# Kitware/pyLiDAR-SLAM

Hardware: NVIDIA H100
Metric: icp_odometry_frames_per_sec (higher is better)
Workload: dtype f32

## Files before the change

pylidar_slam_b200/csrc/context.cu:

```cuda
#include <utility>

#include "internal.cuh"
#include "kdmap_device.cuh"

namespace pls {

long long g_kernel_launches = 0;

void DBuf::reserve(size_t bytes, cudaStream_t s, bool keep) {
    if (bytes <= cap) return;
    size_t want = bytes + bytes / 2 + 256;
    void* np = nullptr;
    PLS_CUDA(cudaStreamSynchronize(s));
    PLS_CUDA(cudaMalloc(&np, want));
    if (p) {
        if (keep) PLS_CUDA(cudaMemcpy(np, p, cap, cudaMemcpyDeviceToDevice));
        PLS_CUDA(cudaFree(p));
    }
    p = np;
    cap = want;
}

void DBuf::reserve_exact(size_t bytes, cudaStream_t s, bool keep) {
    if (bytes <= cap) return;
// ... 148 lines not shown
    cudaEventRecord(e0, ctx->stream);
}

ProfileScope::~ProfileScope() {
    if (e1) cudaEventRecord(e1, ctx->stream);
}

void profile_collect(pls_context* ctx, int which) {
    ProfileSlot& s = ctx->prof[which];
    for (size_t i = 0; i + 1 < s.used; i += 2) {
        float ms = 0.f;
        if (cudaEventElapsedTime(&ms, s.pool[i], s.pool[i + 1]) == cudaSuccess) s.ms += ms;
    }
    s.used = 0;
}

}

using namespace pls;

extern "C" {

const char* pls_version(void) { return "plslam_b200 0.1 (sm_90a)"; }

int pls_host_fingerprint(const void* host_ptr, int64_t num_bytes, uint64_t* out) {
    if (!host_ptr || !out || num_bytes < 0) return PLS_E_INVALID;
    const int64_t words = num_bytes / 8;
    uint64_t h = 0x9E3779B97F4A7C15ull ^ (uint64_t)num_bytes;
    const uint64_t* w = reinterpret_cast<const uint64_t*>(host_ptr);
    const int64_t step = words > 256 ? words / 256 : 1;
    for (int64_t i = 0; i < words; i += step) {
        uint64_t v;
        memcpy(&v, w + i, 8);
        h = (h ^ v) * 0x100000001B3ull;
        h ^= h >> 29;
    }
    if (words > 0) {
        uint64_t v;
        memcpy(&v, w + words - 1, 8);
        h = (h ^ v) * 0x100000001B3ull;
    }
    *out = h;
    return PLS_OK;
}

int pls_launch_count(int64_t* out) {
    if (!out) return PLS_E_INVALID;
    *out = (int64_t)pls::g_kernel_launches;
    return PLS_OK;
}

int pls_config_default(pls_config* c) {
    if (!c) return PLS_E_INVALID;
    memset(c, 0, sizeof(*c));
    c->height = 64;
    c->width = 2048;
    c->up_fov_deg = 3.0f;
    c->down_fov_deg = -24.0f;
    c->local_map_type = PLS_MAP_KDTREE;
    c->local_map_size = 20;
    c->num_neighbors_normals = 10;
    c->normals_kernel_size = 5;
    c->scheme = PLS_SCHEME_DEFAULT;
    c->sigma = 0.5f;
    c->gn_max_iters = 1;
    c->gn_norm_stop = 1e-3f;
    c->max_num_alignments = 100;
    c->threshold_delta_pose = 1e-4f;
    c->threshold_trans = 0.1f;
    c->threshold_rot = 0.3f;
    c->device = 0;
    c->stream = nullptr;
    return PLS_OK;
}

int pls_create(const pls_config* cfg, pls_context** out) {
    if (!cfg || !out) return PLS_E_INVALID;
    *out = nullptr;
    int ndev = 0;
    if (cudaGetDeviceCount(&ndev) != cudaSuccess || ndev <= 0) {
        cudaGetLastError();
        return PLS_E_CUDA;
    }
    if (cfg->device < 0 || cfg->device >= ndev) return PLS_E_INVALID;
    if (cfg->height <= 0 || cfg->width <= 0 || cfg->local_map_size <= 0) return PLS_E_INVALID;
    if (cfg->max_num_alignments < 1 || cfg->max_num_alignments > kMaxAlign) return PLS_E_INVALID;
    if (cfg->num_neighbors_normals < 3 || cfg->num_neighbors_normals + 1 > KD_KMAX_WIDE) return PLS_E_INVALID;
    if (cfg->normals_kernel_size < 1 || cfg->normals_kernel_size > 9 || (cfg->normals_kernel_size % 2) == 0)
        return PLS_E_INVALID;
    pls_context* ctx = new pls_context();
    ctx->cfg = *cfg;
    try {
        PLS_CUDA(cudaSetDevice(cfg->device));
        if (cfg->stream) {
            ctx->stream = (cudaStream_t)cfg->stream;
        } else {
            static const bool prio = !(getenv("PLS_STREAM_PRIORITY") && atoi(getenv("PLS_STREAM_PRIORITY")) == 0);
            int least = 0, greatest = 0;
            PLS_CUDA(cudaDeviceGetStreamPriorityRange(&least, &greatest));
            PLS_CUDA(cudaStreamCreateWithPriority(&ctx->stream, cudaStreamNonBlocking, prio ? greatest : 0));
            ctx->own_stream = true;
        }
        ctx->stream_main = ctx->stream;
        {
            static const bool prio = !(getenv("PLS_STREAM_PRIORITY") && atoi(getenv("PLS_STREAM_PRIORITY")) == 0);
            int least = 0, greatest = 0;
            PLS_CUDA(cudaDeviceGetStreamPriorityRange(&least, &greatest));
            PLS_CUDA(cudaStreamCreateWithPriority(&ctx->stream_map, cudaStreamNonBlocking, prio ? least : 0));
        }
        PLS_CUDA(cudaEventCreateWithFlags(&ctx->ev_map_done, cudaEventDisableTiming));
        ctx->pinned.reserve(kScalarOffset + 256);
        ctx->scalars.reserve(sizeof(FrameResult) + 4096, ctx->stream);
        PLS_CUDA(cudaMemsetAsync(ctx->scalars.p, 0, ctx->scalars.cap, ctx->stream));
        odometry_reset(ctx);
    } catch (const pls::Error& e) {
        fprintf(stderr, "pls_create: %s\n", e.msg.c_str());
        delete ctx;
        return e.code;
    }
    *out = ctx;
    return PLS_OK;
}

int pls_destroy(pls_context* ctx) {
    if (!ctx) return PLS_E_INVALID;
    cudaSetDevice(ctx->cfg.device);
    ctx->upd_pending = false;
    cudaStreamSynchronize(ctx->stream_map);
    cudaStreamSynchronize(ctx->stream_main);
    comm_free(ctx);
    if (ctx->p2p_pending_xchg) cudaFree(ctx->p2p_pending_xchg);
    for (auto& b : ctx->stage_in) b.release();
    for (auto& b : ctx->stage_out) b.release();
    for (auto& b : ctx->tmp) b.release();
    for (auto& b : ctx->next_buf) b.release();
    ctx->pinned.release();
    ctx->scalars.release();
    ctx->sort.keys_alt.release(); ctx->sort.vals_alt.release(); ctx->sort.hist.release();
    ctx->sort.status.release(); ctx->sort.plan.release();
    ctx->sort_map.keys_alt.release(); ctx->sort_map.vals_alt.release(); ctx->sort_map.hist.release();
    ctx->sort_map.status.release(); ctx->sort_map.plan.release();
    ctx->scan.status.release();
    ctx->sel[0].status.release(); ctx->sel[1].status.release(); ctx->input_zbuf.release();
    for (auto& b : ctx->kd.store) b.release();
    ctx->kd.morton.release(); ctx->kd.order.release(); ctx->kd.sorted.release(); ctx->kd.sorted_prev.release(); ctx->kd.normals.release();
    ctx->kd.bbox.release(); ctx->kd.grid_hdr.release(); ctx->kd.cells.release(); ctx->kd.stats.release();
    ctx->kd_worklist.release(); ctx->kd_nn_state.release();
    ctx->pm.vmaps.release(); ctx->pm.nmaps.release(); ctx->pm.poses.release();
    ctx->pm.model_v.release(); ctx->pm.model_n.release(); ctx->pm.zbuf.release();
    for (auto& b : ctx->frame_vmap_buf) b.release();
    for (auto& b : ctx->frame_pts_buf) b.release();
    ctx->queries.release(); ctx->nn_prev.release();
    ctx->partials.release(); ctx->batch_buf.release(); ctx->hyp_buf.release(); ctx->degen_buf.release(); ctx->gs_keys.release(); ctx->gs_vals.release(); ctx->gs_out_xyz.release();
    ctx->gs_out_idx.release();
    for (auto& s : ctx->prof)
        for (auto e : s.pool) cudaEventDestroy(e);
    if (ctx->ev_map_done) cudaEventDestroy(ctx->ev_map_done);
    if (ctx->ev_inputs) cudaEventDestroy(ctx->ev_inputs);
    if (ctx->ev_batch) cudaEventDestroy(ctx->ev_batch);
    if (ctx->ev_icp_done) cudaEventDestroy(ctx->ev_icp_done);
    ctx->gs_host_xyz.release(); ctx->gs_host_idx.release();
    if (ctx->stream_map) cudaStreamDestroy(ctx->stream_map);
    if (ctx->own_stream) cudaStreamDestroy(ctx->stream_main);
    delete ctx;
    return PLS_OK;
}

const char* pls_last_error(pls_context* ctx) { return ctx ? ctx->err.c_str() : "null context"; }

int pls_synchronize(pls_context* ctx) {
    PLS_API_BEGIN(ctx)
    sync_all(ctx);
    PLS_API_END(ctx)
}

int pls_wait_stream(pls_context* ctx, void* other_stream) {
    PLS_API_BEGIN(ctx)
    cudaStream_t other = (cudaStream_t)other_stream;
    if (other != ctx->stream_main) {
        if (!ctx->ev_inputs) PLS_CUDA(cudaEventCreateWithFlags(&ctx->ev_inputs, cudaEventDisableTiming));
        PLS_CUDA(cudaEventRecord(ctx->ev_inputs, other));
        PLS_CUDA(cudaStreamWaitEvent(ctx->stream_main, ctx->ev_inputs, 0));
    }
    PLS_API_END(ctx)
}

int pls_profile_enable(pls_context* ctx, int which, int enable) {
    PLS_API_BEGIN(ctx)
    PLS_REQUIRE(which >= 0 && which < kProfileSlots, "pls_profile_enable: bad slot");
    ctx->prof[which].enabled = enable != 0;
    PLS_API_END(ctx)
}

int pls_profile_read(pls_context* ctx, int which, double* ms_total, int64_t* launches, double* bytes, int reset) {
    PLS_API_BEGIN(ctx)
    PLS_REQUIRE(which >= 0 && which < kProfileSlots, "pls_profile_read: bad slot");
    sync_all(ctx);
    profile_collect(ctx, which);
    ProfileSlot& s = ctx->prof[which];
    if (ms_total) *ms_total = s.ms;
    if (launches) *launches = s.launches;
    if (bytes) *bytes = s.bytes;
    if (reset) {
        s.ms = 0;
        s.launches = 0;
        s.bytes = 0;
    }
    PLS_API_END(ctx)
}

}
```

pylidar_slam_b200/csrc/grid_sample.cu:

```cuda
#include "internal.cuh"
#include "select_device.cuh"

namespace pls {

namespace {

constexpr long long HX = 73856093ll, HY = 19349669ll, HZ = 83492791ll;

constexpr int GS_COMPACT_BITS = 40;

template <typename T>
__global__ void voxel_hash_kernel(const T* __restrict__ xyz, int64_t n, double voxel, long long* __restrict__ coords,
                                  long long* __restrict__ hashes, uint64_t* __restrict__ keys,
                                  uint32_t* __restrict__ vals, uint32_t* __restrict__ overflow = nullptr,
                                  uint32_t stamp = 0, double voxel_y = -1.0, double voxel_z = -1.0) {
    if (voxel_y < 0.0) voxel_y = voxel;
    if (voxel_z < 0.0) voxel_z = voxel;
    for (int64_t i = (int64_t)blockIdx.x * blockDim.x + threadIdx.x; i < n; i += (int64_t)gridDim.x * blockDim.x) {
        double x = (double)xyz[3 * i], y = (double)xyz[3 * i + 1], z = (double)xyz[3 * i + 2];
        long long cx = voxel_coord(x, voxel);
        long long cy = voxel_coord(y, voxel_y);
        long long cz = voxel_coord(z, voxel_z);
        const long long h = (long long)((uint64_t)HX * (uint64_t)cx + (uint64_t)HY * (uint64_t)cy + (uint64_t)HZ * (uint64_t)cz);
        if (coords) {
            coords[3 * i] = cx;
            coords[3 * i + 1] = cy;
            coords[3 * i + 2] = cz;
        }
        if (hashes) hashes[i] = h;
        if (keys) {
            if (overflow) {
                const uint64_t hb = (uint64_t)h + (1ull << (GS_COMPACT_BITS - 1));
                if (hb >> GS_COMPACT_BITS) *overflow = stamp;
                keys[i] = hb & ((1ull << GS_COMPACT_BITS) - 1ull);
            } else {
                keys[i] = (uint64_t)h ^ 0x8000000000000000ull;
            }
            vals[i] = (uint32_t)i;
        }
    }
}

__global__ void head_flags_kernel(const uint64_t* __restrict__ keys, int64_t n, uint8_t* __restrict__ flags) {
    for (int64_t i = (int64_t)blockIdx.x * blockDim.x + threadIdx.x; i < n; i += (int64_t)gridDim.x * blockDim.x)
        flags[i] = (i == 0 || keys[i] != keys[i - 1]) ? 1 : 0;
}

template <typename T>
__global__ void gather_samples_kernel(const T* __restrict__ xyz, const uint32_t* __restrict__ vals,
                                      const uint8_t* __restrict__ flags, const uint32_t* __restrict__ pos, int64_t n,
                                      T* __restrict__ out_xyz, long long* __restrict__ out_idx) {
    for (int64_t i = (int64_t)blockIdx.x * blockDim.x + threadIdx.x; i < n; i += (int64_t)gridDim.x * blockDim.x) {
        if (!flags[i]) continue;
        uint32_t src = vals[i];
        uint32_t dst = pos[i];
        const T x = xyz[3 * (size_t)src], y = xyz[3 * (size_t)src + 1], z = xyz[3 * (size_t)src + 2];
        if (out_idx) out_idx[dst] = (long long)src;
        out_xyz[3 * (size_t)dst] = x;
        out_xyz[3 * (size_t)dst + 1] = y;
        out_xyz[3 * (size_t)dst + 2] = z;
    }
}

__global__ void __launch_bounds__(256)
copy_counted_to_host_kernel(const unsigned char* __restrict__ src_a, unsigned char* __restrict__ dst_a, size_t elem_a,
                            const unsigned char* __restrict__ src_b, unsigned char* __restrict__ dst_b, size_t elem_b,
                            const uint32_t* __restrict__ count_dev) {
    const size_t na = (size_t)*count_dev * elem_a, nb = (size_t)*count_dev * elem_b;
    const size_t va = na / 16, vb = nb / 16;
    const size_t gtid = (size_t)blockIdx.x * blockDim.x + threadIdx.x, stride = (size_t)gridDim.x * blockDim.x;
    for (size_t i = gtid; i < va + vb; i += stride) {
        if (i < va) reinterpret_cast<uint4*>(dst_a)[i] = reinterpret_cast<const uint4*>(src_a)[i];
        else reinterpret_cast<uint4*>(dst_b)[i - va] = reinterpret_cast<const uint4*>(src_b)[i - va];
    }
    if (gtid < 16) {
        size_t o = va * 16 + gtid;
        if (o < na) dst_a[o] = src_a[o];
        o = vb * 16 + gtid;
        if (o < nb) dst_b[o] = src_b[o];
    }
}

template <typename T>
struct GridSampleSelect {
    const uint64_t* keys;
    const uint32_t* vals;
    const T* xyz;
    T* out_xyz;
    long long* out_idx;
    struct State {};
    __device__ __forceinline__ uint32_t flags(int64_t i, State&) const { return (i == 0 || keys[i] != keys[i - 1]) ? 1u : 0u; }
    __device__ __forceinline__ void emit(int64_t i, int, uint32_t dst, const State&) const {
        const uint32_t src = vals[i];
        const T x = xyz[3 * (size_t)src], y = xyz[3 * (size_t)src + 1], z = xyz[3 * (size_t)src + 2];
        if (out_idx) out_idx[dst] = (long long)src;
        out_xyz[3 * (size_t)dst] = x;
        out_xyz[3 * (size_t)dst + 1] = y;
        out_xyz[3 * (size_t)dst + 2] = z;
    }
};

__global__ void voxel_ids_kernel(const uint32_t* __restrict__ vals, const uint8_t* __restrict__ flags,
                                 const uint32_t* __restrict__ pos, int64_t n, long long* __restrict__ ids_out,
                                 uint32_t* __restrict__ starts) {
    for (int64_t i = (int64_t)blockIdx.x * blockDim.x + threadIdx.x; i < n; i += (int64_t)gridDim.x * blockDim.x) {
        const uint32_t id = pos[i] + flags[i] - 1u;
        ids_out[vals[i]] = (long long)id;
        if (flags[i]) starts[id] = (uint32_t)i;
    }
}

template <typename T>
__global__ void __launch_bounds__(256)
voxel_stats_kernel(const T* __restrict__ xyz, const uint32_t* __restrict__ vals, const uint32_t* __restrict__ starts,
                   const uint32_t* __restrict__ count_dev, int64_t n, long long* __restrict__ sizes,
                   T* __restrict__ means, T* __restrict__ covs) {
    const uint32_t V = *count_dev;
    const int lane = threadIdx.x & 31;
    const uint32_t warps = (gridDim.x * blockDim.x) >> 5;
    for (uint32_t v = (blockIdx.x * blockDim.x + threadIdx.x) >> 5; v < V; v += warps) {
        const uint32_t b = starts[v];
        const uint32_t e = (v + 1 < V) ? starts[v + 1] : (uint32_t)n;
        double sx = 0.0, sy = 0.0, sz = 0.0;
        for (uint32_t j = b + lane; j < e; j += 32) {
            const size_t src = vals[j];
            sx += (double)xyz[3 * src];
            sy += (double)xyz[3 * src + 1];
            sz += (double)xyz[3 * src + 2];
        }
        sx = warp_sum(sx); sy = warp_sum(sy); sz = warp_sum(sz);
        const double cnt = (double)(e - b);
        const double mx = sx / cnt, my = sy / cnt, mz = sz / cnt;
        double cxx = 0.0, cxy = 0.0, cxz = 0.0, cyy = 0.0, cyz = 0.0, czz = 0.0;
        for (uint32_t j = b + lane; j < e; j += 32) {
            const size_t src = vals[j];
            const double dx = (double)xyz[3 * src] - mx, dy = (double)xyz[3 * src + 1] - my, dz = (double)xyz[3 * src + 2] - mz;
            cxx += dx * dx; cxy += dx * dy; cxz += dx * dz;
            cyy += dy * dy; cyz += dy * dz; czz += dz * dz;
        }
        cxx = warp_sum(cxx); cxy = warp_sum(cxy); cxz = warp_sum(cxz);
        cyy = warp_sum(cyy); cyz = warp_sum(cyz); czz = warp_sum(czz);
        if (lane == 0) {
            sizes[v] = (long long)(e - b);
            means[3 * (size_t)v] = (T)mx; means[3 * (size_t)v + 1] = (T)my; means[3 * (size_t)v + 2] = (T)mz;
            T* c = covs + 9 * (size_t)v;
            c[0] = (T)cxx; c[1] = (T)cxy; c[2] = (T)cxz;
            c[3] = (T)cxy; c[4] = (T)cyy; c[5] = (T)cyz;
            c[6] = (T)cxz; c[7] = (T)cyz; c[8] = (T)czz;
        }
    }
}

inline int grid_for(int64_t n, int threads = 256) {
    int64_t b = (n + threads - 1) / threads;
    int64_t cap = 8 * kNumSMs;
    return (int)(b < 1 ? 1 : (b > cap ? cap : b));
}

}

template <typename T>
void grid_sample_device(pls_context* ctx, const T* xyz_dev, int64_t n, double voxel, T* out_xyz_dev,
                        long long* out_idx_dev, bool compact, T* host_xyz, long long* host_idx) {
    cudaStream_t st = ctx->stream;
    ProfileScope ps(ctx, 4, (double)n * 3 * sizeof(T));
    ctx->gs_keys.reserve((size_t)n * sizeof(uint64_t), st);
    ctx->gs_vals.reserve((size_t)n * sizeof(uint32_t), st);
    ctx->tmp[1].reserve((size_t)n, st);
    ctx->tmp[2].reserve((size_t)n * sizeof(uint32_t), st);
    if (host_xyz && host_idx && !out_idx_dev) {
        ctx->gs_out_idx.reserve((size_t)n * sizeof(long long), st);
        out_idx_dev = ctx->gs_out_idx.as<long long>();
    }
    auto copy_to_host = [&]() {
        if (!host_xyz || !host_idx) return;
        const size_t bytes = (size_t)n * (3 * sizeof(T) + sizeof(long long));
        copy_counted_to_host_kernel<<<grid_for((int64_t)(bytes / 16)), 256, 0, st>>>(
            reinterpret_cast<const unsigned char*>(out_xyz_dev), reinterpret_cast<unsigned char*>(host_xyz), 3 * sizeof(T),
            reinterpret_cast<const unsigned char*>(out_idx_dev), reinterpret_cast<unsigned char*>(host_idx), sizeof(long long),
            scalar_u32(ctx, SC_GS_COUNT));
        PLS_CHECK_LAUNCH();
    };
    if (compact) {
        ctx->gs_seq += 1;
        if (ctx->gs_seq == 0) ctx->gs_seq = 1;
    }
    voxel_hash_kernel<T><<<grid_for(n), 256, 0, st>>>(xyz_dev, n, voxel, nullptr, nullptr, ctx->gs_keys.as<uint64_t>(),
                                                      ctx->gs_vals.as<uint32_t>(),
                                                      compact ? scalar_u32(ctx, SC_GS_OVERFLOW) : nullptr, ctx->gs_seq);
    PLS_CHECK_LAUNCH();
    uint64_t* sk;
    uint32_t* sv;
    radix_sort_pairs(ctx, ctx->gs_keys.as<uint64_t>(), ctx->gs_vals.as<uint32_t>(), n, compact ? GS_COMPACT_BITS / 8 : 8, &sk, &sv);
    if (n <= SEL_MAX_N) {
        GridSampleSelect<T> op{sk, sv, xyz_dev, out_xyz_dev, out_idx_dev};
        select_launch(ctx, op, n, nullptr, scalar_u32(ctx, SC_GS_COUNT), nullptr);
        copy_to_host();
        return;
    }
    head_flags_kernel<<<grid_for(n), 256, 0, st>>>(sk, n, ctx->tmp[1].as<uint8_t>());
    PLS_CHECK_LAUNCH();
    exclusive_scan_flags(ctx, ctx->tmp[1].as<uint8_t>(), n, ctx->tmp[2].as<uint32_t>(), scalar_u32(ctx, SC_GS_COUNT));
    gather_samples_kernel<T><<<grid_for(n), 256, 0, st>>>(xyz_dev, sv, ctx->tmp[1].as<uint8_t>(),
                                                          ctx->tmp[2].as<uint32_t>(), n, out_xyz_dev, out_idx_dev);
    PLS_CHECK_LAUNCH();
    copy_to_host();
}

template <typename T>
void voxel_statistics_device(pls_context* ctx, const T* xyz_dev, int64_t n, double voxel, long long* coords_dev,
                             long long* hashes_dev, long long* sizes_dev, T* means_dev, T* covs_dev, long long* ids_dev) {
    cudaStream_t st = ctx->stream;
    ctx->gs_keys.reserve((size_t)n * sizeof(uint64_t), st);
    ctx->gs_vals.reserve((size_t)n * sizeof(uint32_t), st);
    ctx->next_buf[1].reserve((size_t)n, st);
    ctx->next_buf[2].reserve((size_t)n * sizeof(uint32_t), st);
    ctx->next_buf[3].reserve((size_t)n * sizeof(uint32_t), st);
    voxel_hash_kernel<T><<<grid_for(n), 256, 0, st>>>(xyz_dev, n, voxel, coords_dev, hashes_dev, ctx->gs_keys.as<uint64_t>(),
                                                      ctx->gs_vals.as<uint32_t>());
    PLS_CHECK_LAUNCH();
    uint64_t* sk;
    uint32_t* sv;
    radix_sort_pairs(ctx, ctx->gs_keys.as<uint64_t>(), ctx->gs_vals.as<uint32_t>(), n, 8, &sk, &sv);
    uint8_t* flags = ctx->next_buf[1].as<uint8_t>();
    uint32_t* pos = ctx->next_buf[2].as<uint32_t>();
    uint32_t* starts = ctx->next_buf[3].as<uint32_t>();
    head_flags_kernel<<<grid_for(n), 256, 0, st>>>(sk, n, flags);
    PLS_CHECK_LAUNCH();
    exclusive_scan_flags(ctx, flags, n, pos, scalar_u32(ctx, SC_GS_COUNT));
    voxel_ids_kernel<<<grid_for(n), 256, 0, st>>>(sv, flags, pos, n, ids_dev, starts);
    PLS_CHECK_LAUNCH();
    voxel_stats_kernel<T><<<grid_for(n * 32), 256, 0, st>>>(xyz_dev, sv, starts, scalar_u32(ctx, SC_GS_COUNT), n, sizes_dev,
                                                           means_dev, covs_dev);
    PLS_CHECK_LAUNCH();
}

namespace {

void grid_sample_count_to_host(pls_context* ctx) {
    uint32_t* words = reinterpret_cast<uint32_t*>(reinterpret_cast<char*>(ctx->pinned.p) + kScalarOffset);
    static_assert(SC_GS_COUNT == 0 && SC_GS_OVERFLOW == 7, "one 32-byte copy covers the count and the overflow stamp");
    PLS_CUDA(cudaMemcpyAsync(words, scalar_u32(ctx, SC_GS_COUNT), 8 * sizeof(uint32_t), cudaMemcpyDeviceToHost, ctx->stream));
}

void grid_sample_launch(pls_context* ctx, const GridSample& g, bool compact) {
    if (!g.f64)
        grid_sample_device<float>(ctx, (const float*)g.xyz, g.n, g.voxel, (float*)g.out_xyz, g.out_idx, compact,
                                  (float*)g.host_xyz, g.host_idx);
    else
        grid_sample_device<double>(ctx, (const double*)g.xyz, g.n, g.voxel, (double*)g.out_xyz, g.out_idx, compact,
                                   (double*)g.host_xyz, g.host_idx);
}

}

void grid_sample_enqueue(pls_context* ctx, const GridSample& g, bool count_to_host) {
    grid_sample_launch(ctx, g, true);
    if (count_to_host) grid_sample_count_to_host(ctx);
}

uint32_t grid_sample_host_count(pls_context* ctx, bool* overflowed) {
    const uint32_t* words = reinterpret_cast<const uint32_t*>(reinterpret_cast<const char*>(ctx->pinned.p) + kScalarOffset);
    *overflowed = ctx->gs_seq != 0 && words[SC_GS_OVERFLOW] == ctx->gs_seq;
    return words[SC_GS_COUNT];
}

uint32_t grid_sample_finish(pls_context* ctx, const GridSample& g) {
    bool overflowed = false;
    const uint32_t count = grid_sample_host_count(ctx, &overflowed);
    if (!overflowed) return count;
    grid_sample_launch(ctx, g, false);
    grid_sample_count_to_host(ctx);
    PLS_CUDA(cudaStreamSynchronize(ctx->stream));
    return grid_sample_host_count(ctx, &overflowed);
}

}

using namespace pls;

extern "C" {

int pls_voxel_hash_xyz(pls_context* ctx, const void* xyz, int is_f64, int64_t n, double voxel_x, double voxel_y, double voxel_z,
                       int64_t* coords_out, int64_t* hashes_out) {
    PLS_API_BEGIN(ctx)
    PLS_REQUIRE(xyz && n > 0 && voxel_x > 0.0 && voxel_y > 0.0 && voxel_z > 0.0, "pls_voxel_hash: need [n,3] points and voxel sizes > 0");
    const size_t esz = is_f64 ? sizeof(double) : sizeof(float);
    const void* d_xyz = to_device(ctx, xyz, (size_t)n * 3 * esz, ctx->stage_in[0]);
    OutArg oc = out_arg(ctx, coords_out, (size_t)n * 3 * sizeof(int64_t), ctx->stage_out[0]);
    OutArg oh = out_arg(ctx, hashes_out, (size_t)n * sizeof(int64_t), ctx->stage_out[1]);
    if (is_f64)
        voxel_hash_kernel<double><<<grid_for(n), 256, 0, ctx->stream>>>((const double*)d_xyz, n, voxel_x, (long long*)oc.dev,
                                                                       (long long*)oh.dev, nullptr, nullptr, nullptr, 0, voxel_y,
                                                                       voxel_z);
    else
        voxel_hash_kernel<float><<<grid_for(n), 256, 0, ctx->stream>>>((const float*)d_xyz, n, voxel_x, (long long*)oc.dev,
                                                                      (long long*)oh.dev, nullptr, nullptr, nullptr, 0, voxel_y,
                                                                      voxel_z);
    PLS_CHECK_LAUNCH();
    finish_out(ctx, oc);
    finish_out(ctx, oh);
    PLS_CUDA(cudaStreamSynchronize(ctx->stream));
    PLS_API_END(ctx)
}

int pls_voxel_hash(pls_context* ctx, const void* xyz, int is_f64, int64_t n, double voxel, int64_t* coords_out,
                   int64_t* hashes_out) {
    return pls_voxel_hash_xyz(ctx, xyz, is_f64, n, voxel, voxel, voxel, coords_out, hashes_out);
}

int pls_grid_sample(pls_context* ctx, const void* xyz, int is_f64, int64_t n, double voxel, void* out_xyz,
                    int64_t* out_idx, int64_t* out_count) {
    PLS_API_BEGIN(ctx)
    PLS_REQUIRE(xyz && out_xyz && out_count && n > 0 && voxel > 0.0, "pls_grid_sample: bad arguments");
    const size_t esz = is_f64 ? sizeof(double) : sizeof(float);
    const void* d_xyz = to_device(ctx, xyz, (size_t)n * 3 * esz, ctx->stage_in[0]);
    OutArg ox = out_arg(ctx, out_xyz, (size_t)n * 3 * esz, ctx->stage_out[0]);
    OutArg oi = out_arg(ctx, out_idx, (size_t)n * sizeof(int64_t), ctx->stage_out[1]);
    const GridSample g{d_xyz, is_f64 != 0, n, voxel, ox.dev, (long long*)oi.dev, nullptr, nullptr};
    grid_sample_enqueue(ctx, g);
    PLS_CUDA(cudaStreamSynchronize(ctx->stream));
    const uint32_t count = grid_sample_finish(ctx, g);
    *out_count = count;
    finish_out(ctx, ox, (size_t)count * 3 * esz);
    finish_out(ctx, oi, (size_t)count * sizeof(int64_t));
    PLS_CUDA(cudaStreamSynchronize(ctx->stream));
    PLS_API_END(ctx)
}

int pls_grid_sample_staged(pls_context* ctx, const void* xyz, int is_f64, int64_t n, double voxel,
                           const void** out_xyz_host, const int64_t** out_idx_host, const void** out_xyz_dev,
                           int64_t* out_count) {
    PLS_API_BEGIN_FRAME(ctx)
    PLS_REQUIRE(xyz && out_xyz_host && out_idx_host && out_count && n > 0 && voxel > 0.0, "pls_grid_sample_staged: bad arguments");
    const size_t esz = is_f64 ? sizeof(double) : sizeof(float);
    const void* d_xyz = to_device(ctx, xyz, (size_t)n * 3 * esz, ctx->stage_in[0]);
    DBuf& dev_xyz = is_f64 ? ctx->stage_out[0] : ctx->gs_out_xyz;
    dev_xyz.reserve((size_t)n * 3 * esz, ctx->stream);
// ... 83 lines not shown
```

pylidar_slam_b200/csrc/internal.cuh:

```cuda
#pragma once
#include <cuda_runtime.h>
#include <math.h>
#include <stddef.h>
#include <stdint.h>
#include <stdio.h>
#include <string.h>

#include <deque>
#include <string>
#include <vector>

#include "../../include/plslam_b200.h"

namespace pls {

constexpr int kNumSMs = 132;
constexpr int NACC = 30;
constexpr int kMaxAlign = 128;
constexpr int kProfileSlots = 16;
constexpr size_t kScalarOffset = 2048;

struct Error {
    int code;
    std::string msg;
// ... 63 lines not shown
struct ProfileSlot {
    bool enabled = false;
    std::vector<cudaEvent_t> pool;
    size_t used = 0;
    double ms = 0.0;
    int64_t launches = 0;
    double bytes = 0.0;
};

struct SortScratch {
    DBuf keys_alt, vals_alt;
    DBuf hist;
    DBuf status;
    DBuf plan;
};

struct ScanScratch {
    DBuf status;
};

struct SelectScratch {
    DBuf status;
    uint32_t epoch = 0;
};

struct KdMap {
    DBuf store[2];
    int cur = 0;
    int64_t count = 0;
    std::deque<int64_t> frame_counts;
    DBuf morton, order;
    DBuf sorted;
    DBuf sorted_prev;
    uint32_t prev_gen = 0;
    DBuf normals;
    DBuf bbox;
    bool bbox_clean = false;
    DBuf grid_hdr;
    DBuf cells;
    DBuf stats;
    size_t table_offset[16] = {};
    uint32_t table_mask[16] = {};
    uint32_t gen = 0;
    int64_t indexed = 0;
    bool valid = false;
    int64_t cap_points = 0;
    int64_t max_frame = 0;
    bool searched = false;
    bool searched_icp = false;
    bool searched_sharded = false;
    bool searched_normals = false;
    uint32_t searched_gen = 0;
    int64_t searched_n = 0;
};

struct ProjMap {
    int K = 0;
    int head = 0;
    DBuf vmaps, nmaps;
    DBuf poses;
    std::vector<float> host_poses;
    DBuf model_v, model_n;
    DBuf zbuf;
    bool valid = false;
    bool zbuf_clean = false;
    int64_t built_lo = 0, built_hi = 0;
};

struct FrameResult {
    float T[16];
    float params[6];
    float losses[kMaxAlign];
    int iters;
    int status;
    int done;
    int pad;
    double last_sums[NACC];
    long long counts[8];
    float first_pt[4];
};

struct Comm;

static_assert(sizeof(FrameResult) <= kScalarOffset, "FrameResult must fit before the scalar slots");

struct KdUpdateWords {
    float X[12];
    float delta[16];
    uint32_t gate;
    uint32_t insert;
    uint32_t skip;
    uint32_t kept;
    uint32_t num_new;
    uint32_t total;
    uint32_t pad[2];
};
constexpr size_t kUpdateOffset = kScalarOffset - 256;
static_assert(sizeof(FrameResult) <= kUpdateOffset && sizeof(KdUpdateWords) <= 256, "KdUpdateWords after FrameResult");

}

struct pls_context {
    pls_config cfg;
    cudaStream_t stream = nullptr;
    cudaStream_t stream_main = nullptr;
    cudaStream_t stream_map = nullptr;
    cudaEvent_t ev_map_done = nullptr;
    cudaEvent_t ev_inputs = nullptr;
    bool map_pending = false;
    bool own_stream = false;
    std::string err;

    pls::DBuf stage_in[4], stage_out[6];
    pls::HBuf pinned;
    pls::DBuf scalars;

    pls::SortScratch sort;
    pls::SortScratch sort_map;
    pls::ScanScratch scan;
    pls::SelectScratch sel[2];
    pls::DBuf input_zbuf;
    bool input_zbuf_clean = false;

    pls::DBuf tmp[8];
    pls::DBuf next_buf[8];

    pls::KdMap kd;
    pls::ProjMap pm;
    int frame_index = 0;
    int last_icp_iters = 0;
    bool icp_result = false;
    bool last_sharded = false;
    int sample_pointcloud = 0;
    float delta_since_update[16];
    pls::DBuf frame_vmap_buf[2];
    pls::DBuf frame_pts_buf[2];
    int frame_slot = 0;
    bool upd_pending = false, upd_insert = false;
    float upd_T[16];
    int upd_slot = 0;
    long long upd_count = 0;
    pls::DBuf queries;
    const float4* query_ptr = nullptr;
    pls::DBuf nn_prev;
    pls::DBuf kd_worklist;
    pls::DBuf kd_nn_state;
    pls::DBuf partials;
    pls::DBuf batch_buf;
    pls::DBuf hyp_buf;
    pls::DBuf degen_buf;
    cudaEvent_t ev_batch = nullptr;
    cudaEvent_t ev_icp_done = nullptr;
    pls::DBuf gs_keys, gs_vals, gs_out_xyz, gs_out_idx;
    uint32_t gs_seq = 0;
    pls::HBuf gs_host_xyz, gs_host_idx;
    int64_t last_query_count = 0;

    pls::Comm* comm = nullptr;
    void* p2p_pending_xchg = nullptr;
    pls::ProfileSlot prof[pls::kProfileSlots];
};

namespace pls {
void flush_map_update(pls_context* ctx);
}

#define PLS_API_BEGIN(ctx)                               \
    if (!(ctx)) return PLS_E_INVALID;                    \
    try {                                                \
        cudaSetDevice((ctx)->cfg.device);                \
        pls::flush_map_update(ctx);

#define PLS_API_BEGIN_FRAME(ctx)                         \
    if (!(ctx)) return PLS_E_INVALID;                    \
    try {                                                \
        cudaSetDevice((ctx)->cfg.device);

#define PLS_API_END(ctx)                                 \
    }                                                    \
    catch (const pls::Error& e) {                        \
        (ctx)->err = e.msg;                              \
        return e.code;                                   \
    }                                                    \
    catch (const std::exception& e) {                    \
        (ctx)->err = e.what();                           \
        return PLS_E_INVALID;                            \
    }                                                    \
    return PLS_OK;

namespace pls {

enum { SC_GS_COUNT = 0, SC_QUERY_COUNT = 1, SC_NAN_COUNT = 2, SC_INSERT_COUNT = 3, SC_PROJ_NC = 4,
       SC_SPARE0 = 5, SC_SPARE1 = 6,
       SC_GS_OVERFLOW = 7,
       SC_KD_COUNTERS = 8,
       SC_KD_LISTS = 16,
       SC_NUM = 32 };

bool is_device_ptr(const void* p);
bool is_device_ptr_uncached(const void* p);
const void* to_device(pls_context* ctx, const void* p, size_t bytes, DBuf& stage);
struct OutArg {
    void* host = nullptr;
    void* dev = nullptr;
    size_t bytes = 0;
};
OutArg out_arg(pls_context* ctx, void* p, size_t bytes, DBuf& stage);
void finish_out(pls_context* ctx, const OutArg& o, size_t bytes_used = (size_t)-1);
void put_out(void* dst, const void* src, size_t bytes);

inline uint32_t* scalar_u32(pls_context* ctx, int i) {
    return reinterpret_cast<uint32_t*>(reinterpret_cast<char*>(ctx->scalars.p) + kScalarOffset) + i;
}
inline FrameResult* frame_result_dev(pls_context* ctx) { return reinterpret_cast<FrameResult*>(ctx->scalars.p); }
inline FrameResult* frame_result_host(pls_context* ctx) { return reinterpret_cast<FrameResult*>(ctx->pinned.p); }
inline KdUpdateWords* kd_update_words_dev(pls_context* ctx) {
    return reinterpret_cast<KdUpdateWords*>(reinterpret_cast<char*>(ctx->scalars.p) + kUpdateOffset);
}
inline const KdUpdateWords* kd_update_words_host(pls_context* ctx) {
    return reinterpret_cast<const KdUpdateWords*>(reinterpret_cast<const char*>(ctx->pinned.p) + kUpdateOffset);
}

void map_stream_begin(pls_context* ctx);
void map_stream_end(pls_context* ctx);
void map_stream_wait(pls_context* ctx);
void sync_all(pls_context* ctx);

struct ProfileScope {
    pls_context* ctx;
    int which;
    cudaEvent_t e0 = nullptr, e1 = nullptr;
    ProfileScope(pls_context* c, int w, double bytes, bool count = true);
    ~ProfileScope();
};
void profile_collect(pls_context* ctx, int which);
inline void profile_credit(pls_context* ctx, int which, int64_t launches, double bytes) {
    if (!ctx->prof[which].enabled) return;
    ctx->prof[which].launches += launches;
    ctx->prof[which].bytes += bytes;
}

void radix_sort_pairs(pls_context* ctx, uint64_t* keys, uint32_t* vals, int64_t n, int num_passes,
                      uint64_t** keys_out, uint32_t** vals_out, int64_t cap_n = 0, const uint32_t* n_dev = nullptr);

void exclusive_scan_flags(pls_context* ctx, const uint8_t* flags, int64_t n, uint32_t* pos_out,
                          uint32_t* total_dev);

#ifdef __CUDACC__
__device__ __forceinline__ float warp_sum(float v) {
#pragma unroll
    for (int o = 16; o > 0; o >>= 1) v += __shfl_xor_sync(0xffffffffu, v, o);
    return v;
}
__device__ __forceinline__ double warp_sum(double v) {
#pragma unroll
    for (int o = 16; o > 0; o >>= 1) v += __shfl_xor_sync(0xffffffffu, v, o);
    return v;
}
__device__ __forceinline__ int float_to_ordered(float f) {
    int i = __float_as_int(f);
    return i >= 0 ? i : i ^ 0x7fffffff;
}
__device__ __forceinline__ float ordered_to_float(int i) {
    return __int_as_float(i >= 0 ? i : i ^ 0x7fffffff);
}
__device__ __forceinline__ long long voxel_coord(double v, double voxel) { return __double2ll_rn(v / voxel); }
#endif

void launch_projection(pls_context* ctx, const float* xyz, const float* channels, int batch, int64_t n,
                       int C, int H, int W, float up, float down, float* out, unsigned long long* zbuf, float fill = 0.f);
void launch_projection_f64(pls_context* ctx, const double* xyz, int64_t n, int H, int W, float up, float down, float* out,
                           unsigned long long* zbuf);
void launch_zbuf_points(pls_context* ctx, const float* xyz, int64_t n, const uint32_t* n_dev, int H, int W, float up, float down,
                        unsigned long long* zbuf);
void launch_normal_map(pls_context* ctx, const float* vmap, int batch, int H, int W, int ksize, float* out);
struct GnParams {
    int scheme;
    double sigma;
};
void kdmap_reset(pls_context* ctx);
void kdmap_update(pls_context* ctx, const float* rel_pose_host, const float* pts_dev, int64_t n,
                  const float* vmap_dev, int H, int W, int64_t known_count);
int64_t kdmap_device_update_bound(const pls_context* ctx, int64_t new_bound);
void kdmap_update_on_device(pls_context* ctx, const float4* fresh_dev, int64_t bound, const KdUpdateWords* upd);
void kdmap_settle_device_update(pls_context* ctx, const KdUpdateWords& w, int local_map_size);
void kdmap_update_packed(pls_context* ctx, const float* rel_pose_host, const float4* fresh_dev, int64_t num_new,
                         bool has_new);
constexpr int KD_BATCH_GRID = 6;
void kdmap_batch_begin(pls_context* lead, pls_context* const* ctxs, const int64_t* query_bounds, int num, cudaStream_t st,
                       int* grid);
void kdmap_batch_iterations(pls_context* lead, int num, cudaStream_t st, const int* grid, int first, int last,
                            double max_distance = HUGE_VAL, double min_eigenvalue = 0.0, double* degen = nullptr);
void kdmap_batch_done(pls_context* lead, int num, cudaStream_t st, int* out);
struct KdScan {
    const float4* queries;
    const uint32_t* nq_dev;
    int64_t bound;
};
void kdmap_hypotheses_begin(pls_context* ctx, const KdScan* scans, int num, cudaStream_t st, int* grid, FrameResult** frs,
                            uint32_t** words);
void kdmap_hypothesis_adopt(pls_context* ctx, const KdScan& scan, int h, cudaStream_t st);
void kdmap_evaluate_batch(pls_context* ctx, int num, cudaStream_t st, const int* grid, double max_d2, double* out);
struct KdScanRows {
    const float* rows;
    int64_t n;
    float4* out;
// ... 41 lines not shown
```

Measured before the change: 2178.

## Replace radix sort in compact grid sampling with bucketed bin sort and select

For compact grid sampling, the multi-pass radix sort plus select is replaced by a three-kernel pipeline. A hash kernel builds a 16-bit bin histogram and scans it into ~1024-element buckets in the last block. A scatter kernel distributes keys into bins. A per-bucket kernel then bitonic-sorts each bucket in shared memory, detects voxel heads, and emits samples using a decoupled look-back prefix. This cuts the number of full-array passes and kernel launches, at the cost of atomic contention, a serialized last-block scan, and a slow fallback path for oversized buckets.

```diff
diff --git a/pylidar_slam_b200/csrc/context.cu b/pylidar_slam_b200/csrc/context.cu
--- a/pylidar_slam_b200/csrc/context.cu
+++ b/pylidar_slam_b200/csrc/context.cu
@@ -324,7 +324,7 @@
     for (auto& b : ctx->frame_pts_buf) b.release();
     ctx->queries.release(); ctx->nn_prev.release();
     ctx->partials.release(); ctx->batch_buf.release(); ctx->hyp_buf.release(); ctx->degen_buf.release(); ctx->gs_keys.release(); ctx->gs_vals.release(); ctx->gs_out_xyz.release();
-    ctx->gs_out_idx.release();
+    ctx->gs_out_idx.release(); ctx->gs_bins.release(); ctx->gs_buckets.release();
     for (auto& s : ctx->prof)
         for (auto e : s.pool) cudaEventDestroy(e);
     if (ctx->ev_map_done) cudaEventDestroy(ctx->ev_map_done);
diff --git a/pylidar_slam_b200/csrc/grid_sample.cu b/pylidar_slam_b200/csrc/grid_sample.cu
--- a/pylidar_slam_b200/csrc/grid_sample.cu
+++ b/pylidar_slam_b200/csrc/grid_sample.cu
@@ -100,6 +100,316 @@
     }
 };
 
+constexpr int GS_BIN_BITS = 16;
+constexpr int GS_BINS = 1 << GS_BIN_BITS;
+constexpr int GS_IDX_BITS = 24;
+constexpr uint64_t GS_IDX_MASK = (1ull << GS_IDX_BITS) - 1ull;
+constexpr uint32_t GS_BUCKET_TARGET = 1024;
+constexpr uint32_t GS_BUCKET_CAP = 4096;
+constexpr int GS_SELECT_THREADS = 512;
+constexpr int GS_SCAN_ITEMS = 8;
+constexpr uint32_t GS_FLAG_AGG = 1u << 30, GS_FLAG_PREFIX = 2u << 30, GS_VALUE_MASK = (1u << 30) - 1u;
+enum { GSW_TICKET = 0, GSW_LO_INV, GSW_HI, GSW_RANGE_LO, GSW_RANGE_HI, GSW_BUCKET_TICKET, GSW_WORDS = 8 };
+
+__device__ __forceinline__ uint32_t gs_ld_volatile(const uint32_t* p) {
+    uint32_t v;
+    asm volatile("ld.volatile.global.u32 %0, [%1];" : "=r"(v) : "l"(p));
+    return v;
+}
+__device__ __forceinline__ void gs_st_volatile(uint32_t* p, uint32_t v) {
+    asm volatile("st.volatile.global.u32 [%0], %1;" ::"l"(p), "r"(v) : "memory");
+}
+
+__device__ __forceinline__ uint32_t gs_block_scan(uint32_t v, uint32_t* s_warp, uint32_t& total) {
+    const int lane = threadIdx.x & 31, warp = threadIdx.x >> 5, warps = blockDim.x >> 5;
+    uint32_t inc = v;
+#pragma unroll
+    for (int o = 1; o < 32; o <<= 1) {
+        const uint32_t t = __shfl_up_sync(0xffffffffu, inc, o);
+        if (lane >= o) inc += t;
+    }
+    if (lane == 31) s_warp[warp] = inc;
+    __syncthreads();
+    uint32_t before = 0, tot = 0;
+    for (int w = 0; w < warps; ++w) {
+        const uint32_t c = s_warp[w];
+        before += w < warp ? c : 0u;
+        tot += c;
+    }
+    __syncthreads();
+    total = tot;
+    return before + inc - v;
+}
+
+template <typename T>
+__global__ void __launch_bounds__(256)
+gs_hash_bins_kernel(const T* __restrict__ xyz, int64_t n, double voxel, uint64_t* __restrict__ keys, uint32_t* bins,
+                    uint32_t* words, uint32_t* __restrict__ bucket_start, uint32_t* __restrict__ status, int num_buckets,
+                    uint32_t* __restrict__ overflow, uint32_t stamp) {
+    __shared__ uint32_t s_lo_inv, s_hi, s_warp[8];
+    __shared__ int s_last;
+    const int tid = threadIdx.x, lane = tid & 31;
+    if (tid == 0) s_lo_inv = s_hi = 0u;
+    __syncthreads();
+    const int64_t stride = (int64_t)gridDim.x * blockDim.x;
+    for (int64_t i = (int64_t)blockIdx.x * blockDim.x + tid; i <= num_buckets; i += stride) status[i] = 0u;
+    for (int64_t base = (int64_t)blockIdx.x * blockDim.x + (tid & ~31); base < n; base += stride) {
+        const int64_t i = base + lane;
+        const bool valid = i < n;
+        uint32_t bin = 0xffffffffu;
+        if (valid) {
+            const long long cx = voxel_coord((double)xyz[3 * i], voxel);
+            const long long cy = voxel_coord((double)xyz[3 * i + 1], voxel);
+            const long long cz = voxel_coord((double)xyz[3 * i + 2], voxel);
+            const uint64_t h = (uint64_t)HX * (uint64_t)cx + (uint64_t)HY * (uint64_t)cy + (uint64_t)HZ * (uint64_t)cz;
+            const uint64_t hb = h + (1ull << (GS_COMPACT_BITS - 1));
+            if (hb >> GS_COMPACT_BITS) *overflow = stamp;
+            const uint64_t k40 = hb & ((1ull << GS_COMPACT_BITS) - 1ull);
+            keys[i] = (k40 << GS_IDX_BITS) | (uint64_t)i;
+            bin = (uint32_t)(k40 >> (GS_COMPACT_BITS - GS_BIN_BITS));
+        }
+        const uint32_t peers = __match_any_sync(0xffffffffu, bin);
+        if (valid && lane == __ffs(peers) - 1) atomicAdd(&bins[bin], (uint32_t)__popc(peers));
+        const uint32_t lo_inv = __reduce_max_sync(0xffffffffu, valid ? (uint32_t)(GS_BINS - 1) - bin : 0u);
+        const uint32_t hi = __reduce_max_sync(0xffffffffu, valid ? bin : 0u);
+        if (lane == 0) {
+            atomicMax(&s_lo_inv, lo_inv);
+            atomicMax(&s_hi, hi);
+        }
+    }
+    __syncthreads();
+    if (tid == 0) {
+        atomicMax(&words[GSW_LO_INV], s_lo_inv);
+        atomicMax(&words[GSW_HI], s_hi);
+    }
+    __threadfence();
+    __syncthreads();
+    if (tid == 0) s_last = atomicAdd(&words[GSW_TICKET], 1u) == gridDim.x - 1;
+    __syncthreads();
+    if (!s_last) return;
+    __threadfence();
+    const uint32_t lo = (uint32_t)(GS_BINS - 1) - __ldcg(&words[GSW_LO_INV]), hi = __ldcg(&words[GSW_HI]);
+    uint32_t carry = 0;
+    for (uint32_t t0 = lo; t0 <= hi; t0 += blockDim.x * GS_SCAN_ITEMS) {
+        const uint32_t b0 = t0 + tid * GS_SCAN_ITEMS;
+        uint32_t c[GS_SCAN_ITEMS], sum = 0;
+#pragma unroll
+        for (int j = 0; j < GS_SCAN_ITEMS; ++j) {
+            c[j] = b0 + j <= hi ? __ldcg(&bins[b0 + j]) : 0u;
+            sum += c[j];
+        }
+        uint32_t total;
+        uint32_t p = carry + gs_block_scan(sum, s_warp, total);
+        carry += total;
+#pragma unroll
+        for (int j = 0; j < GS_SCAN_ITEMS; ++j) {
+            if (b0 + j > hi) break;
+            bins[b0 + j] = p;
+            for (uint32_t k = p / GS_BUCKET_TARGET + 1; k * GS_BUCKET_TARGET <= p + c[j] && k < (uint32_t)num_buckets; ++k)
+                bucket_start[k] = p + c[j];
+            p += c[j];
+        }
+    }
+    if (tid == 0) {
+        bucket_start[0] = 0u;
+        bucket_start[num_buckets] = (uint32_t)n;
+        words[GSW_TICKET] = 0u;
+        words[GSW_LO_INV] = 0u;
+        words[GSW_HI] = 0u;
+        words[GSW_RANGE_LO] = lo;
+        words[GSW_RANGE_HI] = hi;
+        words[GSW_BUCKET_TICKET] = 0u;
+    }
+}
+
+__global__ void __launch_bounds__(256)
+gs_bucket_scatter_kernel(const uint64_t* __restrict__ keys, int64_t n, uint32_t* bins, uint64_t* __restrict__ sorted) {
+    pls_grid_dependency_wait();
+    const int lane = threadIdx.x & 31;
+    const int64_t stride = (int64_t)gridDim.x * blockDim.x;
+    for (int64_t base = (int64_t)blockIdx.x * blockDim.x + (threadIdx.x & ~31); base < n; base += stride) {
+        const int64_t i = base + lane;
+        const bool valid = i < n;
+        const uint64_t k = valid ? keys[i] : 0ull;
+        const uint32_t bin = valid ? (uint32_t)(k >> (GS_IDX_BITS + GS_COMPACT_BITS - GS_BIN_BITS)) : 0xffffffffu;
+        const uint32_t peers = __match_any_sync(0xffffffffu, bin);
+        const int leader = __ffs(peers) - 1;
+        uint32_t pos = 0;
+        if (valid && lane == leader) pos = atomicAdd(&bins[bin], (uint32_t)__popc(peers));
+        pos = __shfl_sync(0xffffffffu, pos, leader) + __popc(peers & ((1u << lane) - 1u));
+        if (valid) sorted[pos] = k;
+    }
+}
+
+__device__ uint32_t gs_bucket_prefix(uint32_t* status, uint32_t b, uint32_t agg) {
+    const int lane = threadIdx.x & 31;
+    if (b == 0) {
+        if (lane == 0) gs_st_volatile(status, GS_FLAG_PREFIX | agg);
+        return 0u;
+    }
+    if (lane == 0) gs_st_volatile(status + b, GS_FLAG_AGG | agg);
+    uint32_t excl = 0;
+    for (int64_t t = (int64_t)b - 1;; t -= 32) {
+        const int64_t j = t - lane;
+        uint32_t v = j >= 0 ? gs_ld_volatile(status + j) : GS_FLAG_PREFIX;
+        while (__any_sync(0xffffffffu, (v >> 30) == 0u))
+            if ((v >> 30) == 0u) v = gs_ld_volatile(status + j);
+        const int first = __ffs(__ballot_sync(0xffffffffu, (v & GS_FLAG_PREFIX) != 0u)) - 1;
+        excl += __reduce_add_sync(0xffffffffu, (first < 0 || lane <= first) ? (v & GS_VALUE_MASK) : 0u);
+        if (first >= 0) break;
+    }
+    if (lane == 0) gs_st_volatile(status + b, GS_FLAG_PREFIX | (excl + agg));
+    return excl;
+}
+
+template <typename T>
+__device__ __forceinline__ void gs_emit(const T* __restrict__ xyz, T* __restrict__ out_xyz, long long* __restrict__ out_idx,
+                                        uint64_t key, uint32_t dst) {
+    const uint32_t src = (uint32_t)(key & GS_IDX_MASK);
+    const T x = xyz[3 * (size_t)src], y = xyz[3 * (size_t)src + 1], z = xyz[3 * (size_t)src + 2];
+    if (out_idx) out_idx[dst] = (long long)src;
+    out_xyz[3 * (size_t)dst] = x;
+    out_xyz[3 * (size_t)dst + 1] = y;
+    out_xyz[3 * (size_t)dst + 2] = z;
+}
+
+__device__ __forceinline__ bool gs_is_head(const uint64_t* k, uint32_t i) {
+    return i == 0 || (k[i] >> GS_IDX_BITS) != (k[i - 1] >> GS_IDX_BITS);
+}
+
+template <typename T>
+__global__ void __launch_bounds__(GS_SELECT_THREADS)
+gs_bucket_select_kernel(uint64_t* sorted, uint64_t* scratch, const uint32_t* __restrict__ bucket_start, uint32_t* status,
+                        uint32_t* words, uint32_t* bins, int num_buckets, const T* __restrict__ xyz, T* __restrict__ out_xyz,
+                        long long* __restrict__ out_idx, uint32_t* __restrict__ count_out) {
+    __shared__ uint64_t s_keys[GS_BUCKET_CAP];
+    __shared__ uint32_t s_warp[GS_SELECT_THREADS / 32];
+    __shared__ uint32_t s_bucket, s_excl;
+    const int tid = threadIdx.x;
+    pls_grid_dependency_wait();
+    if (tid == 0) s_bucket = atomicAdd(&words[GSW_BUCKET_TICKET], 1u);
+    {
+        const uint32_t lo = words[GSW_RANGE_LO], hi = words[GSW_RANGE_HI];
+        for (uint32_t b = lo + blockIdx.x * blockDim.x + tid; b <= hi; b += gridDim.x * blockDim.x) bins[b] = 0u;
+    }
+    __syncthreads();
+    const uint32_t b = s_bucket;
+    const uint32_t s = bucket_start[b], m = bucket_start[b + 1] - s;
+    uint32_t total;
+    if (m <= GS_BUCKET_CAP) {
+        uint32_t P = 1;
+        while (P < m) P <<= 1;
+        for (uint32_t i = tid; i < P; i += blockDim.x) s_keys[i] = i < m ? sorted[s + i] : ~0ull;
+        __syncthreads();
+        for (uint32_t k = 2; k <= P; k <<= 1)
+            for (uint32_t j = k >> 1; j > 0; j >>= 1) {
+                for (uint32_t i = tid; i < P / 2; i += blockDim.x) {
+                    const uint32_t lo = ((i & ~(j - 1)) << 1) | (i & (j - 1)), hi = lo | j;
+                    const uint64_t a = s_keys[lo], c = s_keys[hi];
+                    if ((a > c) == ((lo & k) == 0)) {
+                        s_keys[lo] = c;
+                        s_keys[hi] = a;
+                    }
+                }
+                __syncthreads();
+            }
+        const uint32_t per = (m + blockDim.x - 1) / blockDim.x;
+        const uint32_t i0 = min(tid * per, m), i1 = min(i0 + per, m);
+        uint32_t heads = 0;
+        for (uint32_t i = i0; i < i1; ++i) heads += gs_is_head(s_keys, i);
+        uint32_t dst = gs_block_scan(heads, s_warp, total);
+        if (tid < 32) {
+            const uint32_t e = gs_bucket_prefix(status, b, total);
+            if (tid == 0) s_excl = e;
+        }
+        __syncthreads();
+        dst += s_excl;
+        for (uint32_t i = i0; i < i1; ++i)
+            if (gs_is_head(s_keys, i)) gs_emit(xyz, out_xyz, out_idx, s_keys[i], dst++);
+    } else {
+        uint64_t* a = sorted + s;
+        uint64_t* alt = scratch + s;
+        uint32_t* hist = reinterpret_cast<uint32_t*>(s_keys);
+        uint32_t* warp_cnt = hist + 256;
+        uint64_t kmin = ~0ull, kmax = 0ull;
+        for (uint32_t i = tid; i < m; i += blockDim.x) {
+            const uint64_t k = a[i];
+            kmin = min(kmin, k);
+            kmax = max(kmax, k);
+        }
+        __shared__ unsigned long long s_min, s_max;
+        if (tid == 0) {
+            s_min = ~0ull;
+            s_max = 0ull;
+        }
+        __syncthreads();
+        atomicMin(&s_min, (unsigned long long)kmin);
+        atomicMax(&s_max, (unsigned long long)kmax);
+        __syncthreads();
+        kmin = s_min;
+        const int bits = 64 - __clzll((long long)(s_max - kmin));
+        const int lane = tid & 31, warp = tid >> 5, warps = blockDim.x >> 5;
+        for (int shift = 0; shift < bits; shift += 8) {
+            for (int d = tid; d < 256; d += blockDim.x) hist[d] = 0u;
+            __syncthreads();
+            for (uint32_t i = tid; i < m; i += blockDim.x) atomicAdd(&hist[(uint32_t)((a[i] - kmin) >> shift) & 255u], 1u);
+            __syncthreads();
+            {
+                const uint32_t c = tid < 256 ? hist[tid] : 0u;
+                const uint32_t e = gs_block_scan(c, s_warp, total);
+                if (tid < 256) hist[tid] = e;
+                __syncthreads();
+            }
+            for (uint32_t c0 = 0; c0 < m; c0 += blockDim.x) {
+                for (int w = tid; w < warps * 256; w += blockDim.x) warp_cnt[w] = 0u;
+                __syncthreads();
+                const uint32_t i = c0 + tid;
+                const bool valid = i < m;
+                const uint64_t k = valid ? a[i] : 0ull;
+                const uint32_t d = valid ? ((uint32_t)((k - kmin) >> shift) & 255u) : 256u;
+                const uint32_t peers = __match_any_sync(0xffffffffu, d);
+                const uint32_t rank = __popc(peers & ((1u << lane) - 1u));
+                if (valid && lane == __ffs(peers) - 1) warp_cnt[warp * 256 + d] = __popc(peers);
+                __syncthreads();
+                if (tid < 256) {
+                    uint32_t run = hist[tid];
+                    for (int w = 0; w < warps; ++w) {
+                        const uint32_t c = warp_cnt[w * 256 + tid];
+                        warp_cnt[w * 256 + tid] = run;
+                        run += c;
+                    }
+                    hist[tid] = run;
+                }
+                __syncthreads();
+                if (valid) alt[warp_cnt[warp * 256 + d] + rank] = k;
+                __syncthreads();
+            }
+            uint64_t* t = a;
+            a = alt;
+            alt = t;
+        }
+        uint32_t heads = 0;
+        for (uint32_t i = tid; i < m; i += blockDim.x) heads += gs_is_head(a, i);
+        gs_block_scan(heads, s_warp, total);
+        if (tid < 32) {
+            const uint32_t e = gs_bucket_prefix(status, b, total);
+            if (tid == 0) s_excl = e;
+        }
+        __syncthreads();
+        uint32_t carry = s_excl;
+        for (uint32_t c0 = 0; c0 < m; c0 += blockDim.x) {
+            const uint32_t i = c0 + tid;
+            const bool head = i < m && gs_is_head(a, i);
+            uint32_t chunk;
+            const uint32_t dst = carry + gs_block_scan(head ? 1u : 0u, s_warp, chunk);
+            if (head) gs_emit(xyz, out_xyz, out_idx, a[i], dst);
+            carry += chunk;
+        }
+        total = carry - s_excl;
+    }
+    if (b == (uint32_t)num_buckets - 1 && tid == 0) *count_out = s_excl + total;
+}
+
 __global__ void voxel_ids_kernel(const uint32_t* __restrict__ vals, const uint8_t* __restrict__ flags,
                                  const uint32_t* __restrict__ pos, int64_t n, long long* __restrict__ ids_out,
                                  uint32_t* __restrict__ starts) {
@@ -157,6 +467,31 @@
     return (int)(b < 1 ? 1 : (b > cap ? cap : b));
 }
 
+template <typename T>
+void grid_sample_buckets(pls_context* ctx, const T* xyz_dev, int64_t n, double voxel, T* out_xyz_dev, long long* out_idx_dev) {
+    cudaStream_t st = ctx->stream;
+    const int num_buckets = (int)((n + GS_BUCKET_TARGET - 1) / GS_BUCKET_TARGET);
+    if (!ctx->gs_bins.p) {
+        ctx->gs_bins.reserve_exact((GS_BINS + GSW_WORDS) * sizeof(uint32_t), st);
+        PLS_CUDA(cudaMemsetAsync(ctx->gs_bins.p, 0, (GS_BINS + GSW_WORDS) * sizeof(uint32_t), st));
+    }
+    ctx->gs_buckets.reserve(2 * ((size_t)num_buckets + 1) * sizeof(uint32_t), st);
+    ctx->sort.keys_alt.reserve((size_t)n * sizeof(uint64_t), st);
+    uint32_t* bins = ctx->gs_bins.as<uint32_t>();
+    uint32_t* words = bins + GS_BINS;
+    uint32_t* bucket_start = ctx->gs_buckets.as<uint32_t>();
+    uint32_t* status = bucket_start + num_buckets + 1;
+    uint64_t* keys = ctx->gs_keys.as<uint64_t>();
+    uint64_t* sorted = ctx->sort.keys_alt.as<uint64_t>();
+    gs_hash_bins_kernel<T><<<grid_for(n), 256, 0, st>>>(xyz_dev, n, voxel, keys, bins, words, bucket_start, status,
+                                                        num_buckets, scalar_u32(ctx, SC_GS_OVERFLOW), ctx->gs_seq);
+    PLS_CHECK_LAUNCH();
+    launch_dependent(gs_bucket_scatter_kernel, grid_for(n), 256, st, (const uint64_t*)keys, n, bins, sorted);
+    launch_dependent(gs_bucket_select_kernel<T>, num_buckets, GS_SELECT_THREADS, st, sorted, keys,
+                     (const uint32_t*)bucket_start, status, words, bins, num_buckets, xyz_dev, out_xyz_dev, out_idx_dev,
+                     scalar_u32(ctx, SC_GS_COUNT));
+}
+
 }
 
 template <typename T>
@@ -184,6 +519,11 @@
     if (compact) {
         ctx->gs_seq += 1;
         if (ctx->gs_seq == 0) ctx->gs_seq = 1;
+    }
+    if (compact && n <= SEL_MAX_N) {
+        grid_sample_buckets(ctx, xyz_dev, n, voxel, out_xyz_dev, out_idx_dev);
+        copy_to_host();
+        return;
     }
     voxel_hash_kernel<T><<<grid_for(n), 256, 0, st>>>(xyz_dev, n, voxel, nullptr, nullptr, ctx->gs_keys.as<uint64_t>(),
                                                       ctx->gs_vals.as<uint32_t>(),
diff --git a/pylidar_slam_b200/csrc/internal.cuh b/pylidar_slam_b200/csrc/internal.cuh
--- a/pylidar_slam_b200/csrc/internal.cuh
+++ b/pylidar_slam_b200/csrc/internal.cuh
@@ -239,6 +239,8 @@
     cudaEvent_t ev_batch = nullptr;
     cudaEvent_t ev_icp_done = nullptr;
     pls::DBuf gs_keys, gs_vals, gs_out_xyz, gs_out_idx;
+    pls::DBuf gs_bins;
+    pls::DBuf gs_buckets;
     uint32_t gs_seq = 0;
     pls::HBuf gs_host_xyz, gs_host_idx;
     int64_t last_query_count = 0;
```

New measurement: 2296, median of 6. +5.4%, better.
